# cielavenir/7bgzf

Hardware: NVIDIA B200
Metric: BGZF compress GB/s (uncompressed) (higher is better)
Workload: dtype u8

## Files before the change

7bgzf_b200/b200bgzf.py:

```python
import ctypes
import os

_HERE = os.path.dirname(os.path.abspath(__file__))
LIB_PATH = os.environ.get("B200BGZF_LIB_PATH") or os.path.join(_HERE, "lib7bgzf_b200.so")
HOOK_PATH = os.path.join(_HERE, "7bgzf.so")
APPLET_PATH = os.path.join(_HERE, "7bgzf")

BLOCK_SIZE = 0xFF00
MAX_BLOCK_SIZE = 0x10000
APPEND_EOF = 1
VERIFY = 2
FRAME_MIGZ = 4
E_NOFIT, E_ARG, E_CUDA, E_FORMAT, E_NOSPACE, E_CRC = 1, -1, -2, -3, -4, -5
EOF_BLOCK = bytes.fromhex("1f8b08040000000000ff0600424302001b0003000000000000000000")

EXPORTS = [
    "b200bgzf_create", "b200bgzf_destroy", "b200bgzf_strerror", "b200bgzf_last_error", "b200bgzf_compress_bound",
    "b200bgzf_compress_device", "b200bgzf_compress_host", "b200bgzf_compress_blocks_host", "b200bgzf_inflate_size_host",
    "b200bgzf_inflate_device", "b200bgzf_inflate_host", "b200bgzf_profile", "b200bgzf_launch_count", "b200bgzf_parse_method",
    "b200bgzf_host_alloc", "b200bgzf_host_free", "b200bgzf_member_header", "b200bgzf_compress_host_index", "b200bgzf_gzi_format",
    "b200bgzf_multi_create", "b200bgzf_multi_destroy", "b200bgzf_multi_count", "b200bgzf_multi_ctx", "b200bgzf_shard_blocks",
    "b200bgzf_multi_compress_bound", "b200bgzf_multi_compress_host", "b200bgzf_multi_inflate_host",
    "b200bgzf_pieces_gap_bytes", "b200bgzf_compress_pieces_host", "b200bgzf_crc32_combine", "b200bgzf_container_plan",
    "b200bgzf_container_head", "b200bgzf_container_bound", "b200bgzf_container_frame", "b200bgzf_container_compress_host",
# ... 107 lines not shown
    if rc != 0:
        raise B200BgzfError(rc, "container plan")
    return bs.value, sp


def container_frame(kind, param, stream, piece_off, piece_crc, in_bytes, lib=None):
    lib = lib or load()
    n = len(piece_off)
    head = lib.b200bgzf_container_head(kind, n)
    buf = bytearray(head + len(stream) + 64 + 40 * (n + 1))
    buf[head : head + len(stream)] = stream
    off = (ctypes.c_uint64 * max(n, 1))(*piece_off)
    crc = (ctypes.c_uint32 * max(n, 1))(*piece_crc)
    total = lib.b200bgzf_container_frame(kind, param, _addr(buf), len(buf), len(stream), off, crc, n, in_bytes)
    return bytes(buf[:total])


def _addr(buf):
    if isinstance(buf, int):
        return buf
    if isinstance(buf, bytes):
        return ctypes.cast(ctypes.c_char_p(buf), ctypes.c_void_p).value
    if hasattr(buf, "ctypes"):
        return buf.ctypes.data
    if hasattr(buf, "data_ptr"):
        return buf.data_ptr()
    return ctypes.addressof((ctypes.c_char * len(buf)).from_buffer(buf))


class Codec:

    def __init__(self, device=-1, path=LIB_PATH):
        self.lib = load(path)
        h = ctypes.c_void_p()
        rc = self.lib.b200bgzf_create(ctypes.byref(h), device)
        if rc != 0:
            raise B200BgzfError(rc, self.lib.b200bgzf_strerror(rc).decode())
        self.h = h

    def close(self):
        if self.h:
            self.lib.b200bgzf_destroy(self.h)
            self.h = None

    def __del__(self):
        try:
            self.close()
        except Exception:
            pass

    def _check(self, rc, ok=(0,)):
        if rc not in ok:
            raise B200BgzfError(rc, self.lib.b200bgzf_strerror(rc).decode() + " / " + self.lib.b200bgzf_last_error(self.h).decode())
        return rc

    def bound(self, n, block_size=BLOCK_SIZE):
        return self.lib.b200bgzf_compress_bound(n, block_size)

    def compress(self, data, level=6, block_size=BLOCK_SIZE, eof=True, flags=0):
        out = bytearray(self.bound(len(data), block_size))
        n = ctypes.c_size_t()
        self._check(self.lib.b200bgzf_compress_host(self.h, _addr(data) if len(data) else None, len(data), block_size, level,
                                                    _addr(out), len(out), ctypes.byref(n), (APPEND_EOF if eof else 0) | flags))
        return bytes(out[: n.value])

    def compress_pieces(self, data, spec, level=6, block_size=BLOCK_SIZE):
        nb = (len(data) + block_size - 1) // block_size
        cap = self.bound(len(data), block_size) + self.lib.b200bgzf_pieces_gap_bytes(len(data), block_size, ctypes.byref(spec))
        out = bytearray(cap)
        off = (ctypes.c_uint64 * max(nb, 1))()
        crc = (ctypes.c_uint32 * max(nb, 1))()
        n = ctypes.c_size_t()
        self._check(self.lib.b200bgzf_compress_pieces_host(self.h, _addr(data) if len(data) else None, len(data), block_size, level,
                                                           ctypes.byref(spec), _addr(out), len(out), ctypes.byref(n), off, crc, max(nb, 1)))
        return bytes(out[: n.value]), list(off[:nb]), list(crc[:nb])

    def container(self, kind, data, level=6, param=0):
        out = bytearray(self.lib.b200bgzf_container_bound(kind, param, len(data)))
        n = ctypes.c_size_t()
        self._check(self.lib.b200bgzf_container_compress_host(self.h, kind, param, _addr(data) if len(data) else None, len(data), level,
                                                              _addr(out), len(out), ctypes.byref(n)))
        return bytes(out[: n.value])

    def container_inflate(self, kind, blob, flags=0):
        total = ctypes.c_size_t()
        rc = self.lib.b200bgzf_container_inflate_size(kind, _addr(blob), len(blob), ctypes.byref(total), None)
        if rc != 0:
            raise B200BgzfError(rc, "container size")
        total = total.value
        out = bytearray(max(total, 1))
        n = ctypes.c_size_t()
        self._check(self.lib.b200bgzf_container_inflate_host(self.h, kind, _addr(blob), len(blob), _addr(out), len(out), ctypes.byref(n), flags))
        return bytes(out[: n.value])

    def inflate_units(self, blob, units, out_bytes, flags=0, want_crc=False):
        arr = (Unit * len(units))(*[Unit(*u) for u in units])
        out = bytearray(max(out_bytes, 1))
        n = ctypes.c_size_t()
        crc = (ctypes.c_uint32 * max(len(units), 1))() if want_crc else None
        self._check(self.lib.b200bgzf_inflate_units_host(self.h, _addr(blob), len(blob), arr, len(units), _addr(out), len(out), ctypes.byref(n), flags, crc))
        return (bytes(out[: n.value]), list(crc[: len(units)])) if want_crc else bytes(out[: n.value])

    def compress_indexed(self, data, level=6, block_size=BLOCK_SIZE, eof=True):
        nb = (len(data) + block_size - 1) // block_size
        out = bytearray(self.bound(len(data), block_size))
        off = (ctypes.c_uint64 * max(nb, 1))()
        n = ctypes.c_size_t()
        self._check(self.lib.b200bgzf_compress_host_index(self.h, _addr(data) if len(data) else None, len(data), block_size, level,
                                                          _addr(out), len(out), ctypes.byref(n), APPEND_EOF if eof else 0, off, nb))
        return bytes(out[: n.value]), list(off[:nb])

    def compress_into(self, src_addr, nbytes, dst_addr, dst_cap, level=6, block_size=BLOCK_SIZE, eof=True):
        n = ctypes.c_size_t()
        self._check(self.lib.b200bgzf_compress_host(self.h, src_addr, nbytes, block_size, level, dst_addr, dst_cap, ctypes.byref(n),
                                                    APPEND_EOF if eof else 0))
        return n.value

    def inflate(self, data, flags=0):
        total, nm = ctypes.c_size_t(), ctypes.c_size_t()
        self._check(self.lib.b200bgzf_inflate_size_host(_addr(data), len(data), ctypes.byref(total), ctypes.byref(nm)))
        out = bytearray(max(total.value, 1))
        n = ctypes.c_size_t()
        self._check(self.lib.b200bgzf_inflate_host(self.h, _addr(data), len(data), _addr(out), len(out), ctypes.byref(n), flags))
        return bytes(out[: n.value])

    def inflate_into(self, src_addr, nbytes, dst_addr, dst_cap, flags=0):
        n = ctypes.c_size_t()
        self._check(self.lib.b200bgzf_inflate_host(self.h, src_addr, nbytes, dst_addr, dst_cap, ctypes.byref(n), flags))
        return n.value

    def compress_blocks(self, payloads, level=6, caps=None):
        nb = len(payloads)
        srcs = (ctypes.c_void_p * nb)(*[_addr(p) if len(p) else None for p in payloads])
        slen = (ctypes.c_uint32 * nb)(*[len(p) for p in payloads])
        bufs = [bytearray(MAX_BLOCK_SIZE) for _ in range(nb)]
        dsts = (ctypes.c_void_p * nb)(*[_addr(b) for b in bufs])
        dlen = (ctypes.c_size_t * nb)(*(caps or [MAX_BLOCK_SIZE] * nb))
        st = (ctypes.c_int * nb)()
        rc = self.lib.b200bgzf_compress_blocks_host(self.h, srcs, slen, dsts, dlen, st, nb, level)
        self._check(rc, ok=(0, 1))
        return [bytes(bufs[i][: dlen[i]]) if st[i] == 0 else None for i in range(nb)], list(st)

    def compress_device(self, d_in, nbytes, d_out, out_cap, level=6, block_size=BLOCK_SIZE, eof=True, stream=None):
        n = ctypes.c_size_t()
        self._check(self.lib.b200bgzf_compress_device(self.h, d_in, nbytes, block_size, level, d_out, out_cap, ctypes.byref(n),
                                                      APPEND_EOF if eof else 0, stream))
        return n.value

    def inflate_device(self, d_in, nbytes, d_out, out_cap, flags=0, stream=None):
        n = ctypes.c_size_t()
        self._check(self.lib.b200bgzf_inflate_device(self.h, d_in, nbytes, d_out, out_cap, ctypes.byref(n), flags, stream))
        return n.value

    def profile(self, enable=True, reset=True):
        arr = (ctypes.c_ulonglong * 32)()
        self._check(self.lib.b200bgzf_profile(self.h, 1 if enable else 0, arr, 32, 1 if reset else 0))
        return list(arr)

    def launches(self):
        return self.lib.b200bgzf_launch_count(self.h)


class MultiCodec:

    def __init__(self, devices, path=LIB_PATH):
        self.lib = load(path)
        h = ctypes.c_void_p()
        arr = (ctypes.c_int * len(devices))(*devices)
        rc = self.lib.b200bgzf_multi_create(ctypes.byref(h), arr, len(devices))
        if rc != 0:
            raise B200BgzfError(rc, self.lib.b200bgzf_strerror(rc).decode())
        self.h = h

    def close(self):
        if self.h:
            self.lib.b200bgzf_multi_destroy(self.h)
            self.h = None

    def count(self):
        return self.lib.b200bgzf_multi_count(self.h)

    def bound(self, n, block_size=BLOCK_SIZE):
        return self.lib.b200bgzf_multi_compress_bound(self.h, n, block_size)

    def _check(self, rc):
        if rc != 0:
            raise B200BgzfError(rc, self.lib.b200bgzf_strerror(rc).decode())

    def compress_into(self, src_addr, nbytes, dst_addr, dst_cap, level=6, block_size=BLOCK_SIZE, eof=True, flags=0):
        n = ctypes.c_size_t()
        self._check(self.lib.b200bgzf_multi_compress_host(self.h, src_addr, nbytes, block_size, level, dst_addr, dst_cap, ctypes.byref(n),
                                                          (APPEND_EOF if eof else 0) | flags))
        return n.value

    def compress(self, data, level=6, block_size=BLOCK_SIZE, eof=True, flags=0):
        out = bytearray(self.bound(len(data), block_size))
        n = self.compress_into(_addr(data) if len(data) else None, len(data), _addr(out), len(out), level, block_size, eof, flags)
        return bytes(out[:n])

    def container(self, kind, data, level=6, param=0):
        out = bytearray(self.lib.b200bgzf_multi_container_bound(self.h, kind, param, len(data)))
        n = ctypes.c_size_t()
        self._check(self.lib.b200bgzf_multi_container_compress_host(self.h, kind, param, _addr(data) if len(data) else None, len(data), level,
                                                                    _addr(out), len(out), ctypes.byref(n)))
        return bytes(out[: n.value])

    def inflate_into(self, src_addr, nbytes, dst_addr, dst_cap, flags=0):
        n = ctypes.c_size_t()
        self._check(self.lib.b200bgzf_multi_inflate_host(self.h, src_addr, nbytes, dst_addr, dst_cap, ctypes.byref(n), flags))
        return n.value

    def inflate(self, data, flags=0):
        total, nm = ctypes.c_size_t(), ctypes.c_size_t()
        self._check(self.lib.b200bgzf_inflate_size_host(_addr(data), len(data), ctypes.byref(total), ctypes.byref(nm)))
        out = bytearray(max(total.value, 1))
        n = self.inflate_into(_addr(data), len(data), _addr(out), len(out), flags)
        return bytes(out[:n])


def shard_blocks(nblocks, shard, nshards, lib=None):
    lib = lib or load()
    a, b = ctypes.c_uint64(), ctypes.c_uint64()
    lib.b200bgzf_shard_blocks(nblocks, shard, nshards, ctypes.byref(a), ctypes.byref(b))
    return a.value, b.value


def member_header(data, lib=None):
    lib = lib or load()
    n = ctypes.c_uint64()
    h = lib.b200bgzf_member_header(_addr(data), len(data), ctypes.byref(n))
    return h, n.value


def gzi_format(caddr, uaddr, lib=None):
    lib = lib or load()
    n = len(caddr)
    ca, ua = (ctypes.c_uint64 * max(n, 1))(*caddr), (ctypes.c_uint64 * max(n, 1))(*uaddr)
    buf = bytearray(8 + 16 * max(n - 1, 0))
    w = lib.b200bgzf_gzi_format(ca, ua, n, _addr(buf), len(buf))
    return bytes(buf[:w])
```

7bgzf_b200/csrc/bgzf_compress.cu:

```cuda
#include <cuda_runtime.h>
#include <stdint.h>

#include <atomic>
#include <cstring>

#include "bgzf_block.h"
#include "bgzf_kernels.h"

#define SM_DATA 0u
#define SM_REGA (BG_DATA_BYTES)
#define SM_REGB (SM_REGA + 131072u)
#define SM_CRCTAB (SM_REGB + 32768u)
#define SM_LITFLAG (SM_CRCTAB + 1024u)
#define SM_SCAL (SM_LITFLAG + 256u)
#define SM_MBAR (SM_SCAL + 4u * BG_S_COUNT)
#define SM_FRONTIER (SM_MBAR + 8u)
#define SM_SCAN (SM_MBAR + 16u)
#define SM_READY (SM_SCAN + 4u * 36u)
#define SM_TOTAL (SM_READY + 128u)

extern "C" size_t bgzf_compress_smem_bytes(void) { return SM_TOTAL; }

__device__ __forceinline__ uint32_t smem_u32(const void *p) { return (uint32_t)__cvta_generic_to_shared(p); }

__device__ __forceinline__ void mbar_init(uint64_t *bar, uint32_t count)
{
    asm volatile("mbarrier.init.shared::cta.b64 [%0], %1;" ::"r"(smem_u32(bar)), "r"(count) : "memory");
}
__device__ __forceinline__ void mbar_expect_tx(uint64_t *bar, uint32_t bytes)
{
    asm volatile("mbarrier.arrive.expect_tx.shared::cta.b64 _, [%0], %1;" ::"r"(smem_u32(bar)), "r"(bytes) : "memory");
}
__device__ __forceinline__ void mbar_wait(uint64_t *bar, uint32_t parity)
{
    asm volatile(
        "{\n"
        ".reg .pred p;\n"
        "WAIT_%=:\n"
        "mbarrier.try_wait.parity.shared::cta.b64 p, [%0], %1;\n"
        "@p bra DONE_%=;\n"
        "bra WAIT_%=;\n"
        "DONE_%=:\n"
        "}\n" ::"r"(smem_u32(bar)), "r"(parity) : "memory");
}
__device__ __forceinline__ void tma_load_1d(void *dst_smem, const void *src_gmem, uint32_t bytes, uint64_t *bar)
{
    asm volatile("cp.async.bulk.shared::cluster.global.mbarrier::complete_tx::bytes [%0], [%1], %2, [%3];" ::"r"(smem_u32(dst_smem)),
                 "l"(src_gmem), "r"(bytes), "r"(smem_u32(bar))
                 : "memory");
}
__device__ __forceinline__ void fence_proxy_async()
{
    asm volatile("fence.proxy.async.shared::cta;" ::: "memory");
}

__device__ __forceinline__ unsigned hash_peers(uint32_t h, bool valid)
{
    unsigned peers = __ballot_sync(0xffffffffu, valid);
#pragma unroll
    for (int k = 0; k < BG_HASH_BITS; k++) {
        const uint32_t bit = (h >> k) & 1u;
        const unsigned b = __ballot_sync(0xffffffffu, bit != 0);
        peers &= b ^ (bit - 1u);
    }
    return peers;
}

__device__ __forceinline__ void build_peers_phase(const BgCtx &c, uint4 *notes, uint32_t lane, uint32_t warp, uint32_t nwarps, uint32_t first,
                                                  uint32_t step, uint4 *xprev, volatile uint8_t *ready)
{
    const uint32_t n = c.n, hb = c.scal[BG_S_HBYTES];
    const unsigned lt = (1u << lane) - 1u;
    const uint32_t ntiles = (n + 511u) >> 9;
    for (uint32_t tile = first + step * warp; tile < ntiles; tile += step * nwarps) {
        uint32_t w[4] = { 0xffffffffu, 0xffffffffu, 0xffffffffu, 0xffffffffu };
#pragma unroll
        for (uint32_t g = 0; g < 16; g++) {
            const uint32_t base = tile * 512u + g * 32u;
            if (base >= n) break;
            const uint32_t p = base + lane;
            const bool valid = p + hb <= n;
            const uint32_t h = valid ? bg_hash(c.dataw, p, hb) : BG_NOPOS;
            const unsigned peers = hash_peers(h, valid);
            uint32_t link = h;
            if (valid) {
                const unsigned lower = peers & lt;
                if (lower) {
                    link = base + (31u - (uint32_t)__clz(lower));
                } else {
                    const uint32_t note = 31u - (uint32_t)__clz(peers);
                    w[g >> 2] = (w[g >> 2] & ~(0xffu << (8 * (g & 3)))) | (note << (8 * (g & 3)));
                }
            }
            if (p < n) c.prev[p] = (uint16_t)link;
        }
        notes[tile * 32u + lane] = make_uint4(w[0], w[1], w[2], w[3]);
        if (xprev) {
            __syncwarp();
            const uint4 *ts = (const uint4 *)(c.prev + tile * 512u);
            xprev[tile * 64u + lane] = ts[lane];
            xprev[tile * 64u + 32u + lane] = ts[32u + lane];
        }
        if (ready) {
            __threadfence_block();
            __syncwarp();
            if (lane == 0) ready[tile] = 1;
        }
    }
}

__device__ __forceinline__ void import_peer_tiles(const BgCtx &c, const uint4 *xprev, uint32_t t, uint32_t rank, uint32_t parts)
{
    const uint32_t pieces = ((c.n + 511u) >> 9) * 64u;
    uint4 *dst = (uint4 *)c.prev;
    for (uint32_t i = t; i < pieces; i += BG_THREADS)
        if ((i >> 6) % parts != rank) dst[i] = __ldcg(xprev + i);
}

#define BG_LINKERS 4u
__device__ __forceinline__ void build_link_phase(const BgCtx &c, const uint4 *notes, uint32_t warp, uint32_t lane, volatile uint32_t *turn,
                                                 volatile uint8_t *ready)
{
    const uint32_t n = c.n;
    const uint32_t ntiles = (n + 511u) >> 9;
    volatile uint16_t *vhead = c.head;
    for (uint32_t tile = warp; tile < ntiles; tile += BG_LINKERS) {
        if (ready) {
            while (!ready[tile]) __nanosleep(40);
            __threadfence_block();
        }
        const uint4 cur = __ldcg(notes + tile * 32u + lane);
        const uint32_t w[4] = { cur.x, cur.y, cur.z, cur.w };
        uint32_t hs[16];
#pragma unroll
        for (uint32_t g = 0; g < 16; g++) {
            const uint32_t note = (w[g >> 2] >> (8 * (g & 3))) & 0xffu;
            hs[g] = note != 0xffu ? (uint32_t)c.prev[tile * 512u + g * 32u + lane] : 0xffffffffu;
        }
        while (*turn != tile) {}
        __threadfence_block();
        uint16_t old[16];
#pragma unroll
        for (uint32_t g = 0; g < 16; g++) {
            const uint32_t h = hs[g];
            if (h != 0xffffffffu) {
                const uint32_t note = (w[g >> 2] >> (8 * (g & 3))) & 31u;
                old[g] = vhead[h];
                vhead[h] = (uint16_t)(tile * 512u + g * 32u + note);
            }
        }
        __threadfence_block();
        __syncwarp();
        if (lane == 0) *turn = tile + 1;
#pragma unroll
        for (uint32_t g = 0; g < 16; g++)
            if (hs[g] != 0xffffffffu) c.prev[tile * 512u + g * 32u + lane] = old[g];
    }
}


__device__ __forceinline__ void mark_remote(uint32_t *local_word, uint32_t owner, uint32_t bits)
{
    uint32_t raddr;
    asm volatile("mapa.shared::cluster.u32 %0, %1, %2;" : "=r"(raddr) : "r"(smem_u32(local_word)), "r"(owner));
    asm volatile("red.relaxed.cluster.shared::cluster.or.b32 [%0], %1;" ::"r"(raddr), "r"(bits) : "memory");
}

template <bool SPLIT>
__device__ __forceinline__ void mark_bits(uint32_t *mark, uint32_t word, uint32_t bits, uint32_t own, uint32_t parts)
{
    BG_ASSERT(word < 2064u);
    if (!SPLIT) {
        atomicOr(&mark[word], bits);
        return;
    }
    const uint32_t owner = word % parts;
    if (owner == own) atomicOr(&mark[word], bits);
    else mark_remote(&mark[word], owner, bits);
    if (bits & 0xC0000000u) {
        const uint32_t next = (word + 1u) % parts;
        if (next == own) atomicOr(&mark[word], bits & 0xC0000000u);
        else if (next != owner) mark_remote(&mark[word], next, bits & 0xC0000000u);
    }
}

template <bool SPLIT, bool H3>
__device__ __forceinline__ void search_nearest_t(const BgCtx &c, uint32_t t, uint32_t own, uint32_t parts)
{
    const uint32_t n = c.n, lane = t & 31u;
    uint32_t *elig = (uint32_t *)(c.regb + BG_B_TODO), *mark = (uint32_t *)(c.regb + BG_B_MARK);
    const BgSearchPrm sp = bg_search_prm(c);
    if (sp.depth <= 1) {
        const uint32_t hist1 = bg_f_hist(c);
        for (uint32_t p = t; p < n; p += BG_THREADS) {
            if (SPLIT && (p >> 5) % parts != own) continue;
            bool deep;
            uint32_t target;
            c.R[p] = p < hist1 ? 0u : bg_nearest_t<H3>(c, sp, p, &deep, &target);
        }
        return;
    }
    const bool opt = c.prm.opt_passes > 0;
    const uint32_t hist = bg_f_hist(c);
    if (t == 0 && own == 0) mark_bits<SPLIT>(mark, hist >> 5, 1u << (hist & 31u), own, parts);
    for (uint32_t p0 = t - lane; p0 < n; p0 += BG_THREADS) {
        const uint32_t word = p0 >> 5;
        BG_ASSERT(word < 2048u);
        if (SPLIT && word % parts != own) continue;
        const uint32_t p = p0 + lane;
        if (p0 + 32u <= hist) {
            c.R[p] = 0;
            if (opt) ((uint4 *)c.cand)[p] = make_uint4(0u, 0u, 0u, 0u);
            continue;
        }
        bool deep = false;
        uint32_t target = p + 1, r = 0;
        const bool live = p < n && p >= hist;
        if (live) r = bg_nearest_t<H3>(c, sp, p, &deep, &target);
        if (p < n) c.R[p] = r;
        if (opt) {
            if (p < n) {
                const uint32_t k = r ? bg_off_bin(bg_mw_off(r)) : 4u;
                ((uint4 *)c.cand)[p] = make_uint4(k == 0 ? r : 0u, k == 1 ? r : 0u, k == 2 ? r : 0u, k == 3 ? r : 0u);
            }
            const unsigned em = __ballot_sync(0xffffffffu, deep);
            if (lane == 0) elig[word] = em;
            continue;
        }
        const bool lit = live && target == p + 1;
        const unsigned lm = __ballot_sync(0xffffffffu, lit), em = __ballot_sync(0xffffffffu, deep);
        const uint32_t before = __shfl_up_sync(0xffffffffu, target, 1);
        if (lane == 0) {
            elig[word] = em;
            if (lm << 1) mark_bits<SPLIT>(mark, word, lm << 1, own, parts);
            if (lm >> 31) mark_bits<SPLIT>(mark, word + 1, 1u, own, parts);
        }
        if (live && !lit && (lane == 0 || before != target)) mark_bits<SPLIT>(mark, target >> 5, 1u << (target & 31u), own, parts);
    }
}

template <bool SPLIT>
__device__ __forceinline__ void search_nearest(const BgCtx &c, uint32_t t, uint32_t own, uint32_t parts)
{
    if (c.scal[BG_S_HBYTES] == 3) search_nearest_t<SPLIT, true>(c, t, own, parts);
    else search_nearest_t<SPLIT, false>(c, t, own, parts);
}

template <bool H3>
__device__ __forceinline__ void drain_queue(const BgCtx &c, const uint32_t *queue, uint32_t from, uint32_t count, uint32_t lane)
{
    if (lane < count) {
        const uint32_t e = queue[from + lane];
        const uint32_t p = e >> 16, q = e & 0xffffu;
        BG_ASSERT(p < c.n && q < p && p - q <= 32768u);
        const uint32_t v = bg_deep_extend(c, H3, p, q);
        if (v) {
            atomicMax(&c.R[p], v);
            if (c.cand) atomicMax(&c.cand[4u * p + bg_off_bin(p - q)], v);
        }
    }
}

template <bool H3>
__device__ __forceinline__ void deep_batch(const BgCtx &c, uint32_t *queue, uint32_t &cnt, uint32_t p, bool active, uint32_t lane)
{
    uint32_t q = BG_NOPOS, b1 = 3, tail = 0;
    int depth = (int)c.scal[BG_S_DEPTH] - 1;
    const unsigned lt = (1u << lane) - 1u;
    uint32_t tmask = 0xffffffffu;
    if (active) {
        const uint32_t r1 = __ldcg(c.R + p);
        b1 = r1 ? r1 >> 16 : 3u;
        tmask = bg_tail_mask(H3, r1);
        tail = bg_ld32(c.dataw, p + b1 - 3u) & tmask;
        q = c.prev[c.prev[p]];
    }
    bool live = active && depth > 0 && bg_in_window(p, q);
    const uint32_t f4 = H3 && active ? bg_ld32(c.dataw, p) : 0u;
    int cap = 4 * depth;
    while (__any_sync(0xffffffffu, live)) {
#pragma unroll
        for (uint32_t k = 0; k < BG_SCAN_CHUNK_SHALLOW; k++) {
            bool pass = false;
            const uint32_t qc = q;
            if (live) {
                const uint32_t qn = c.prev[q];
                pass = (bg_ld32(c.dataw, q + b1 - 3u) & tmask) == tail;
                if (!H3 || bg_ld32(c.dataw, q) == f4) depth--;
                if (H3) cap--;
                q = qn;
                live = depth > 0 && (!H3 || cap > 0) && bg_in_window(p, q);
            }
            const unsigned m = __ballot_sync(0xffffffffu, pass);
            if (m) {
                BG_ASSERT(cnt + __popc(m) <= BG_QUEUE_WORDS_SHALLOW);
                if (pass) queue[cnt + __popc(m & lt)] = (p << 16) | qc;
                cnt += __popc(m);
            }
        }
        if (cnt >= 32u) {
            __syncwarp();
            do {
                cnt -= 32u;
                drain_queue<H3>(c, queue, cnt, 32u, lane);
            } while (cnt >= 32u);
            __syncwarp();
            if (live) {
                const uint32_t r = __ldcg(c.R + p);
                if ((r >> 16) > b1) {
// ... 242 lines not shown

__device__ __forceinline__ uint32_t chunk_class(const BgCtx &c, uint32_t ch)
{
    if (ch * BG_CHUNK >= c.n) return 0u;
    const uint32_t *sc = (const uint32_t *)(c.stepcode + ch * BG_CHUNK);
    uint32_t zeros = 0;
#pragma unroll
    for (uint32_t k = 0; k < BG_CHUNK / 4u; k++) {
        const uint32_t v = sc[k];
        zeros += __popc((v - 0x01010101u) & ~v & 0x80808080u);
    }
    return zeros >= 64u ? 7u : zeros >> 3;
}

__device__ __forceinline__ void chunk_order_count(const BgCtx &c, uint32_t t, uint32_t &cls, uint32_t &rank)
{
    const uint32_t lane = t & 31u, warp = t >> 5;
    uint32_t *cnt = (uint32_t *)(c.regb + BG_B_CLASSCNT);
    cls = chunk_class(c, t);
    rank = 0;
#pragma unroll
    for (uint32_t k = 0; k < 8u; k++) {
        const unsigned m = __ballot_sync(0xffffffffu, cls == k);
        if (cls == k) rank = __popc(m & ((1u << lane) - 1u));
        if (lane == k) cnt[k * 32u + warp] = __popc(m);
    }
}

__device__ __forceinline__ void chunk_order_scan(const BgCtx &c, uint32_t t)
{
    if (t >= 32u) return;
    uint32_t *cnt = (uint32_t *)(c.regb + BG_B_CLASSCNT);
    uint32_t v[8], sum = 0;
#pragma unroll
    for (uint32_t k = 0; k < 8u; k++) { v[k] = cnt[t * 8u + k]; sum += v[k]; }
    uint32_t inc = sum;
    for (int d = 1; d < 32; d <<= 1) {
        const uint32_t y = __shfl_up_sync(0xffffffffu, inc, d);
        if (t >= (uint32_t)d) inc += y;
    }
    uint32_t run = inc - sum;
#pragma unroll
    for (uint32_t k = 0; k < 8u; k++) { cnt[t * 8u + k] = run; run += v[k]; }
}

__device__ __forceinline__ void chunk_order_place(const BgCtx &c, uint32_t t, uint32_t cls, uint32_t rank)
{
    const uint32_t *cnt = (const uint32_t *)(c.regb + BG_B_CLASSCNT);
    BG_ASSERT(cls < 8u && cnt[cls * 32u + (t >> 5)] + rank < BG_MAX_CHUNKS);
    ((uint16_t *)(c.regb + BG_B_PERM))[cnt[cls * 32u + (t >> 5)] + rank] = (uint16_t)t;
}

__device__ __forceinline__ void bitonic_sort_512(uint32_t *keys, uint32_t t)
{
    for (uint32_t k = 2; k <= 512; k <<= 1) {
        for (uint32_t j = k >> 1; j > 0; j >>= 1) {
            if (t < 512) {
                uint32_t x = t ^ j;
                if (x > t) {
                    uint32_t a = keys[t], b = keys[x];
                    bool up = (t & k) == 0;
                    if ((a > b) == up) { keys[t] = b; keys[x] = a; }
                }
            }
            __syncthreads();
        }
    }
}

__device__ __forceinline__ uint32_t block_exclusive_scan_1024(uint32_t *v, uint32_t *scratch, uint32_t t)
{
    const uint32_t lane = t & 31u, warp = t >> 5;
    uint32_t x = v[t], inc = x;
    for (int d = 1; d < 32; d <<= 1) {
        uint32_t y = __shfl_up_sync(0xffffffffu, inc, d);
        if (lane >= (uint32_t)d) inc += y;
    }
    if (lane == 31) scratch[warp] = inc;
    __syncthreads();
    if (warp == 0) {
        uint32_t w = scratch[lane], winc = w;
        for (int d = 1; d < 32; d <<= 1) {
            uint32_t y = __shfl_up_sync(0xffffffffu, winc, d);
            if (lane >= (uint32_t)d) winc += y;
        }
        scratch[lane] = winc - w;
        if (lane == 31) scratch[32] = winc;
    }
    __syncthreads();
    v[t] = scratch[warp] + inc - x;
    uint32_t total = scratch[32];
    __syncthreads();
    return total;
}

__device__ __forceinline__ void gather_member(const uint32_t *src, uint32_t n, uint8_t *dst, uint32_t t, uint32_t nthr)
{
    const uint32_t head = (uint32_t)((4u - ((uintptr_t)dst & 3u)) & 3u);
    if (n <= head + 4) {
        for (uint32_t i = t; i < n; i += nthr) dst[i] = (uint8_t)(__ldcg(src + (i >> 2)) >> (8u * (i & 3u)));
        return;
    }
    if (t < head) dst[t] = (uint8_t)(__ldcg(src) >> (8u * t));
    const uint32_t words = (n - head) >> 2;
    uint32_t *dw = (uint32_t *)(dst + head);
    const uint32_t sh = head * 8u;
    for (uint32_t i = t; i < words; i += nthr)
        dw[i] = __funnelshift_r(__ldcg(src + i), __ldcg(src + i + 1), sh);
    const uint32_t done = head + words * 4u;
    if (t < n - done) dst[done + t] = (uint8_t)(__ldcg(src + ((done + t) >> 2)) >> (8u * ((done + t) & 3u)));
}

__device__ __forceinline__ uint32_t block_exclusive_scan_1024(uint32_t *v, uint32_t *scratch, uint32_t t);

__device__ __forceinline__ void fused_compaction(const BgzfCompressArgs &a, uint32_t *v, uint32_t *scratch, uint32_t t)
{
    uint64_t carry = *a.gather_total;
    for (uint32_t start = 0; start < a.nblocks; start += 1024u) {
        const uint32_t i = start + t;
        v[t] = i < a.nblocks ? __ldcg(a.out_len + i) : 0u;
        __syncthreads();
        const uint32_t total = block_exclusive_scan_1024(v, scratch, t);
        if (i < a.nblocks) a.gather_off[i] = carry + v[t];
        carry += total;
        __syncthreads();
    }
    if (t == 0) *a.gather_total = carry;
    __syncthreads();
    const uint32_t grp = t >> 8, gt = t & 255u;
    for (uint32_t b = grp; b < a.nblocks; b += BG_THREADS / 256u) {
        BG_ASSERT(__ldcg(a.out_len + b) <= BG_SLOT_BYTES && a.gather_off[b] + __ldcg(a.out_len + b) <= carry);
        gather_member((const uint32_t *)(a.slots + (size_t)b * BG_SLOT_BYTES), __ldcg(a.out_len + b), a.gather_out + a.gather_off[b], gt, 256u);
    }
}

#define PROF_MARK(i)                                                        \
    do {                                                                    \
        if (prof && t == 0) {                                               \
            long long now_ = clock64();                                     \
            atomicAdd((unsigned long long *)&prof[i], (unsigned long long)(now_ - tprev_)); \
            tprev_ = now_;                                                  \
        }                                                                   \
    } while (0)

template <bool SPLIT>
__device__ __forceinline__ void compress_blocks(BgzfCompressArgs &a)
{
    extern __shared__ __align__(128) uint8_t smem[];
    const uint32_t t = threadIdx.x, T = BG_THREADS;
    uint64_t *mbar = (uint64_t *)(smem + SM_MBAR);
    uint32_t *scan_scratch = (uint32_t *)(smem + SM_SCAN);
    unsigned long long *prof = a.prof;
    long long tprev_ = prof ? clock64() : 0;

    BgCtx c;
    c.dataw = (uint32_t *)(smem + SM_DATA);
    c.prev = (uint16_t *)(smem + SM_REGA);
    c.stepcode = smem + SM_REGA;
    c.jump8 = smem + SM_REGA + 65536u;
    c.offarr = (uint16_t *)(smem + SM_REGA + 65536u);
    c.head = (uint16_t *)(smem + SM_REGB);
    c.regb = smem + SM_REGB;
    c.crctab = (uint32_t *)(smem + SM_CRCTAB);
    c.litflag = smem + SM_LITFLAG;
    c.scal = (uint32_t *)(smem + SM_SCAL);
    const uint32_t crank = SPLIT ? cluster_rank() : 0u, csize = SPLIT ? cluster_size() : 1u;
    const uint32_t unit = SPLIT ? blockIdx.x / csize : blockIdx.x;
    uint32_t *const unit_scratch = a.scratch + (size_t)unit * (SPLIT ? BGZF_SCRATCH_WORDS + BGZF_SPLIT_EXTRA_WORDS : BGZF_SCRATCH_WORDS);
    c.R = unit_scratch;
    c.cand = a.cand ? a.cand + (size_t)unit * (4u * BG_MAX_BLOCK) : nullptr;
    c.crcpow = a.crcpow;
    c.prm = a.prm;
    c.frame = bg_frame(a.hdr_bytes ? a.hdr_bytes : 18u, 8u, 1u, 0u);
    c.perm = (const uint16_t *)(smem + SM_REGB + BG_B_PERM);

    if (t < 256) c.crctab[t] = a.crctab[t];
    if (t == 0) {
        mbar_init(mbar, 1);
        asm volatile("fence.mbarrier_init.release.cluster;" ::: "memory");
    }
    __syncthreads();
    uint32_t parity = 0;

    for (uint32_t b = unit; b < a.nblocks; b += SPLIT ? a.nblocks : gridDim.x) {
        const uint8_t *src;
        uint32_t n;
        if (a.in_off) {
            src = a.in + a.in_off[b];
            n = a.in_len[b];
        } else {
            const uint64_t off = (uint64_t)b * a.block_size;
            src = a.in + off;
            const uint64_t rem = a.in_bytes - off;
            n = rem < a.block_size ? (uint32_t)rem : a.block_size;
        }
        c.out = (uint32_t *)(a.slots + (size_t)b * BG_SLOT_BYTES);
        if (a.piece_mode) {
            const uint64_t gb = a.piece_base + b;
            const bool first = gb % a.member_blocks == 0, last = (gb + 1) % a.member_blocks == 0 || gb + 1 == a.piece_total;
            uint32_t hist = 0;
            if (a.history && !first && !a.in_off) {
                const uint64_t in_member = (gb % a.member_blocks) * a.block_size, in_buffer = (uint64_t)a.lead + (uint64_t)b * a.block_size;
                uint64_t h = in_member < in_buffer ? in_member : in_buffer;
                if (h > a.history) h = a.history;
                hist = (uint32_t)h - (uint32_t)h % BG_HISTORY_STEP;
            }
            src -= hist;
            n += hist;
            c.frame = bg_frame(first ? a.head_gap : 0u, last ? a.tail_gap : 0u, last && !a.no_final ? 1u : 0u, 1u, hist);
        }
        c.n = n;

        const bool aligned = (((uintptr_t)src) & 15u) == 0;
        const uint32_t bulk = aligned ? (n & ~15u) : 0u;
        if (bulk) {
            if (t == 0) {
                fence_proxy_async();
                mbar_expect_tx(mbar, bulk);
                tma_load_1d(smem + SM_DATA, src, bulk, mbar);
            }
        }
        for (uint32_t i = bulk + t; i < n; i += T)
            smem[SM_DATA + i] = src[i];
        bg_phase_init(c, t, T);
        if (bulk) {
            mbar_wait(mbar, parity);
            parity ^= 1u;
        }
        __syncthreads();
        PROF_MARK(0);

        bg_phase_scan(c, t, T);
        __syncthreads();
        bg_phase_count(c, t, T);
        __syncthreads();
        bg_phase_settle(c, t, T);
        __syncthreads();
        PROF_MARK(1);
        PROF_MARK(2);
        uint4 *hi = (uint4 *)(c.R + BG_MAX_BLOCK + 32);
        if (SPLIT) {
            uint4 *xprev = (uint4 *)(unit_scratch + BGZF_SCRATCH_WORDS);
            build_peers_phase(c, hi, t & 31u, t >> 5, BG_THREADS / 32u, crank, csize, xprev, nullptr);
            cluster_sync();
            import_peer_tiles(c, xprev, t, crank, csize);
            __syncthreads();
            PROF_MARK(3);
            if (t < 32u * BG_LINKERS) build_link_phase(c, hi, t >> 5, t & 31u, &c.scal[BG_S_WLIST], nullptr);
        } else {
            volatile uint8_t *ready = (volatile uint8_t *)(smem + SM_READY);
            if (t < 128u) ready[t] = 0;
            __syncthreads();
            if (t < 32u * BG_LINKERS) build_link_phase(c, hi, t >> 5, t & 31u, &c.scal[BG_S_WLIST], ready);
            else build_peers_phase(c, hi, t & 31u, (t >> 5) - BG_LINKERS, BG_THREADS / 32u - BG_LINKERS, 0u, 1u, nullptr, ready);
        }
        __syncthreads();
        PROF_MARK(10);
        {
            bg_phase_search_clear(c, t, T);
            if (SPLIT) cluster_sync();
            else __syncthreads();
            search_nearest<SPLIT>(c, t, crank, csize);
            if (SPLIT) cluster_sync();
            else __syncthreads();
            PROF_MARK(21);
            if (c.scal[BG_S_DEPTH] > 1) {
                bg_phase_search_todo(c, t, T, crank, csize);
                __syncthreads();
                const bool h3 = c.scal[BG_S_HBYTES] == 3;
                if (c.scal[BG_S_DEPTH] <= 24u) {
                    if (h3) search_deep_batches<true>(c, t, crank, csize);
                    else search_deep_batches<false>(c, t, crank, csize);
                } else {
                    if (h3) search_deep<true>(c, t, crank, csize);
                    else search_deep<false>(c, t, crank, csize);
                }
            }
        }
        if (SPLIT) {
            cluster_sync();
            if (crank) return;
        }
        __syncthreads();
        PROF_MARK(4);
        for (int pass = 0; pass <= c.prm.opt_passes; pass++) {
            if (pass == 0) {
                bg_phase_accept(c, t, T);
            } else {
                bg_phase_costs(c, t, T);
                __syncthreads();
                dp_segment_warp(c, t >> 5, t & 31u, (uint32_t *)(smem + SM_REGA + 65536u) + (t >> 5) * BG_DP_RING);
            }
            __syncthreads();
            if (bg_f_hist(c)) {
                bg_phase_history_steps(c, t, T);
                __syncthreads();
            }
            PROF_MARK(15);
            bg_phase_jump(c, t, T);
            __syncthreads();
            PROF_MARK(5);
            bg_phase_walk_clear(c, t, T);
            bg_phase_clear_freq(c, t, T);
            __syncthreads();
            bg_phase_walk_mark(c, t, T);
            __syncthreads();
            bg_phase_walk_list(c, t, T);
            __syncthreads();
            PROF_MARK(16);
            bg_phase_walk_a(c, t, T);
            __syncthreads();
            PROF_MARK(17);
            bg_phase_walk_b(c, t, T);
            uint32_t ccls, crnk;
            chunk_order_count(c, t, ccls, crnk);
            __syncthreads();
            PROF_MARK(18);
            bg_phase_walk_c(c, t, T);
            chunk_order_scan(c, t);
            __syncthreads();
            chunk_order_place(c, t, ccls, crnk);
            __syncthreads();
            PROF_MARK(6);
            bg_phase_tally(c, t, T);
            __syncthreads();
            bg_phase_lkeys(c, t, T);
            __syncthreads();
            PROF_MARK(7);
            bitonic_sort_512((uint32_t *)(c.regb + BG_B_KEYS), t);
            PROF_MARK(11);
            bg_phase_huff_prep(c, t, T);
            __syncthreads();
            bg_phase_huff(c, t, T);
            __syncthreads();
            bg_phase_huff_depth(c, t, T);
            __syncthreads();
            bg_phase_huff_fix(c, t, T);
            __syncthreads();
            bg_phase_huff_assign(c, t, T);
            __syncthreads();
            PROF_MARK(12);
        }
        bg_phase_hdr1(c, t, T);
        __syncthreads();
        bg_phase_hdr2(c, t, T);
        __syncthreads();
        bg_phase_hdr3(c, t, T);
        __syncthreads();
        const uint32_t nitems = block_exclusive_scan_1024((uint32_t *)(c.regb + BG_B_CBITS), scan_scratch, t);
        bg_phase_hdr4(c, t, T);
        __syncthreads();
        bg_phase_hdr4b(c, t, T);
        __syncthreads();
        bg_phase_hdr5(c, t, T, nitems);
        __syncthreads();
        PROF_MARK(13);
        bg_phase_decide_b(c, t, T);
        __syncthreads();
        bg_phase_codes_a(c, t, T);
        __syncthreads();
        bg_phase_codes_b(c, t, T);
        __syncthreads();
        bg_phase_codes_c(c, t, T);
        __syncthreads();
        bg_phase_tabs(c, t, T);
        __syncthreads();
        PROF_MARK(8);
        bg_phase_hdr_bits(c, t, T);
        bg_phase_sizes(c, t, T);
        __syncthreads();
        PROF_MARK(19);
        block_exclusive_scan_1024((uint32_t *)(c.regb + BG_B_CBITS), scan_scratch, t);
        block_exclusive_scan_1024((uint32_t *)(c.regb + BG_B_IOFF), scan_scratch, t);
        PROF_MARK(20);
        bg_phase_zero_out(c, t, T);
        __syncthreads();
        PROF_MARK(14);
        bg_phase_emit(c, t, T);
        if (t == 0) {
            const uint32_t st = c.scal[BG_S_STATUS];
            a.out_len[b] = st ? 0u : bg_f_hdr(c) + c.scal[BG_S_PAYLOAD] + bg_f_trl(c);
            if (a.crc_out) a.crc_out[b] = c.scal[BG_S_CRC];
            a.status[b] = st;
            if (st) atomicOr(a.err_flag, 1u);
        }
        fence_proxy_async();
        __syncthreads();
        PROF_MARK(9);
    }
    if (!SPLIT && a.gather_out) {
        __threadfence();
        __syncthreads();
        if (t == 0) scan_scratch[35] = atomicAdd(a.done_count, 1u) == gridDim.x - 1u ? 1u : 0u;
        __syncthreads();
        if (scan_scratch[35]) {
            __threadfence();
            fused_compaction(a, (uint32_t *)(smem + SM_REGB), scan_scratch, t);
        }
    }
}

__global__ void __launch_bounds__(BG_THREADS, 1)
bgzf_compress_kernel(BgzfCompressArgs a)
{
    compress_blocks<false>(a);
}

__global__ void __launch_bounds__(BG_THREADS, 1)
bgzf_compress_split_kernel(BgzfCompressArgs a)
{
    compress_blocks<true>(a);
}

__global__ void __launch_bounds__(1024, 1)
bgzf_scan_kernel(const uint32_t *len, uint64_t *off, uint32_t nmax, const uint64_t *count_dev, const uint64_t *base_dev,
                 uint64_t *total_out)
{
// ... 125 lines not shown
```

7bgzf_b200/csrc/bgzf_kernels.h:

```cpp
#ifndef BGZF_KERNELS_H
#define BGZF_KERNELS_H
#include <cuda_runtime.h>
#include <stdint.h>

#include "bgzf_block.h"

#define BGZF_SCRATCH_WORDS (65536u + 32u + 16384u + 32u)
#define BGZF_SPLIT_EXTRA_WORDS 32768u
#define BGZF_SPLIT_MAX 8
#define BGZF_PROF_SLOTS 32

struct BgzfCompressArgs {
    const uint8_t *in;
    const uint64_t *in_off;
    const uint32_t *in_len;
    uint64_t in_bytes;
    uint32_t block_size;
    uint32_t nblocks;
    uint32_t hdr_bytes;
    BgParams prm;
    uint8_t *slots;
    uint32_t *out_len;
    uint32_t *status;
    uint32_t *err_flag;
    uint32_t *scratch;
    uint32_t *cand;
    const uint32_t *crctab;
    const uint32_t *crcpow;
    unsigned long long *prof;
    uint8_t *gather_out;
    uint64_t *gather_off;
    uint64_t *gather_total;
    uint32_t *done_count;
    uint32_t piece_mode;
    uint32_t member_blocks;
    uint64_t piece_base;
    uint64_t piece_total;
    uint32_t head_gap;
    uint32_t tail_gap;
    uint32_t no_final;
    uint32_t *crc_out;
    uint32_t history;
    uint32_t lead;
};

struct BgzfInflateArgs {
    const uint8_t *in;
    const uint64_t *in_off;
    const uint64_t *out_off;
    const uint32_t *hdr_len;
    const uint32_t *msize;
    const uint32_t *unit_isize;
    uint32_t *unit_crc;
    uint32_t nblocks;
    uint8_t *out;
    uint32_t *status;
    uint32_t *err_flag;
    int verify_crc;
    const uint32_t *crctab;
    const uint32_t *crcpow;
};

struct BgzfIndexWork {
    uint32_t max_blocks;
    uint32_t *tile_count;
    uint64_t *tile_off;
    uint64_t *cand_off;
    uint32_t *jump, *jump2;
    uint32_t *reach;
    uint64_t *pick_idx;
    uint64_t *in_off;
    uint64_t *out_off;
    uint32_t *isize;
    uint64_t *ncand, *nmembers, *out_bytes;
    uint32_t *status;
};

#ifdef __cplusplus
extern "C" {
#endif
size_t bgzf_compress_smem_bytes(void);
cudaError_t bgzf_launch_compress(const BgzfCompressArgs *a, int grid, cudaStream_t stream);
cudaError_t bgzf_launch_compress_split(const BgzfCompressArgs *a, int csize, cudaStream_t stream);
cudaError_t bgzf_launch_scan(const uint32_t *len, uint64_t *off, uint32_t nmax, const uint64_t *count_dev,
                             const uint64_t *base_dev, uint64_t *total_out, cudaStream_t stream);
cudaError_t bgzf_launch_compact(const uint8_t *slots, const uint32_t *len, uint64_t *off, uint32_t nblocks, uint8_t *out,
                                uint64_t *total, int append_eof, cudaStream_t stream);
cudaError_t bgzf_launch_deliver(const uint8_t *slots, const uint32_t *len, const uint64_t *out_off, uint8_t *host_out, uint32_t n,
                                cudaStream_t stream);
size_t bgzf_index_tiles(uint64_t in_bytes);
#define BGZF_INDEX_LAUNCHES 8
cudaError_t bgzf_launch_index(const uint8_t *in, uint64_t in_bytes, const BgzfIndexWork *w, cudaStream_t stream);
cudaError_t bgzf_launch_inflate(const BgzfInflateArgs *a, cudaStream_t stream);
#ifdef __cplusplus
}
#endif
#endif
```

Before: 29.37.

## Streamline hash-chain linking with branchless sink writes and acquire/release turn handoff

The hash-peer ballot loop becomes inline PTX that fuses the bit test, vote and mask update. A branchless masked hash covers all supported widths. The serialized linker phase packs hash and position into one op word and sends invalid entries to a dummy sink slot in shared memory, so every lane stores unconditionally. Acquire/release shared-memory ops replace the volatile spin plus thread fences on the turn counter. Optional per-tile profiling counters are also added, which widens the profile buffer and puts extra branches in the hot path.

```diff
diff --git a/7bgzf_b200/b200bgzf.py b/7bgzf_b200/b200bgzf.py
--- a/7bgzf_b200/b200bgzf.py
+++ b/7bgzf_b200/b200bgzf.py
@@ -283,9 +283,9 @@
         self._check(self.lib.b200bgzf_inflate_device(self.h, d_in, nbytes, d_out, out_cap, ctypes.byref(n), flags, stream))
         return n.value
 
-    def profile(self, enable=True, reset=True):
-        arr = (ctypes.c_ulonglong * 32)()
-        self._check(self.lib.b200bgzf_profile(self.h, 1 if enable else 0, arr, 32, 1 if reset else 0))
+    def profile(self, enable=True, reset=True, slots=32):
+        arr = (ctypes.c_ulonglong * slots)()
+        self._check(self.lib.b200bgzf_profile(self.h, 1 if enable else 0, arr, slots, 1 if reset else 0))
         return list(arr)
 
     def launches(self):
diff --git a/7bgzf_b200/csrc/bgzf_compress.cu b/7bgzf_b200/csrc/bgzf_compress.cu
--- a/7bgzf_b200/csrc/bgzf_compress.cu
+++ b/7bgzf_b200/csrc/bgzf_compress.cu
@@ -59,17 +59,30 @@
     unsigned peers = __ballot_sync(0xffffffffu, valid);
 #pragma unroll
     for (int k = 0; k < BG_HASH_BITS; k++) {
-        const uint32_t bit = (h >> k) & 1u;
-        const unsigned b = __ballot_sync(0xffffffffu, bit != 0);
-        peers &= b ^ (bit - 1u);
+        asm volatile("{\n\t.reg .pred p;\n\t.reg .b32 b, t;\n\t"
+                     "and.b32 t, %1, %2;\n\t"
+                     "setp.ne.u32 p, t, 0;\n\t"
+                     "vote.sync.ballot.b32 b, p, 0xffffffff;\n\t"
+                     "selp.b32 t, -1, 0, p;\n\t"
+                     "lop3.b32 %0, %0, b, t, 0x90;\n\t}"
+                     : "+r"(peers)
+                     : "r"(h), "r"(1u << k));
     }
     return peers;
 }
 
+__device__ __forceinline__ uint32_t hash_any_width(const uint32_t *dataw, uint32_t p, uint32_t m0, uint32_t m1)
+{
+    const uint32_t v0 = bg_ld32(dataw, p) & m0, v1 = bg_ld32(dataw, p + 4u) & m1;
+    return ((v0 * 0x1E35A7BDu) ^ (v1 * 0x9E3779B1u)) >> (32 - BG_HASH_BITS);
+}
+
 __device__ __forceinline__ void build_peers_phase(const BgCtx &c, uint4 *notes, uint32_t lane, uint32_t warp, uint32_t nwarps, uint32_t first,
-                                                  uint32_t step, uint4 *xprev, volatile uint8_t *ready)
+                                                  uint32_t step, uint4 *xprev, volatile uint8_t *ready, unsigned long long *prof, long long t0)
 {
     const uint32_t n = c.n, hb = c.scal[BG_S_HBYTES];
+    const uint32_t m0 = hb == 3 ? 0xffffffu : 0xffffffffu, m1 = hb == 8 ? 0xffffffffu : hb == 5 ? 0xffu : 0u;
+    BG_ASSERT(hb == 3 || hb == 4 || hb == 5 || hb == 8);
     const unsigned lt = (1u << lane) - 1u;
     const uint32_t ntiles = (n + 511u) >> 9;
     for (uint32_t tile = first + step * warp; tile < ntiles; tile += step * nwarps) {
@@ -80,7 +93,7 @@
             if (base >= n) break;
             const uint32_t p = base + lane;
             const bool valid = p + hb <= n;
-            const uint32_t h = valid ? bg_hash(c.dataw, p, hb) : BG_NOPOS;
+            const uint32_t h = valid ? hash_any_width(c.dataw, p, m0, m1) : BG_NOPOS;
             const unsigned peers = hash_peers(h, valid);
             uint32_t link = h;
             if (valid) {
@@ -105,6 +118,7 @@
             __threadfence_block();
             __syncwarp();
             if (lane == 0) ready[tile] = 1;
+            if (prof && lane == 0) atomicAdd(&prof[BGZF_PROF_READY + tile], (unsigned long long)(clock64() - t0));
         }
     }
 }
@@ -118,43 +132,63 @@
 }
 
 #define BG_LINKERS 4u
+#define BG_LINK_SINK (SM_SCAN + 4u * 33u - SM_REGB)
+__device__ __forceinline__ uint32_t ld_acquire_cta(const volatile uint32_t *p)
+{
+    uint32_t v;
+    asm volatile("ld.acquire.cta.shared::cta.u32 %0, [%1];" : "=r"(v) : "r"(smem_u32((const void *)p)) : "memory");
+    return v;
+}
+__device__ __forceinline__ void st_release_cta(volatile uint32_t *p, uint32_t v)
+{
+    asm volatile("st.release.cta.shared::cta.u32 [%0], %1;" ::"r"(smem_u32((const void *)p)), "r"(v) : "memory");
+}
 __device__ __forceinline__ void build_link_phase(const BgCtx &c, const uint4 *notes, uint32_t warp, uint32_t lane, volatile uint32_t *turn,
-                                                 volatile uint8_t *ready)
+                                                 volatile uint8_t *ready, unsigned long long *prof, long long t0)
 {
     const uint32_t n = c.n;
     const uint32_t ntiles = (n + 511u) >> 9;
-    volatile uint16_t *vhead = c.head;
+    volatile uint8_t *vhead = (volatile uint8_t *)c.head;
+    static_assert(BG_LINK_SINK >= 2u * BG_HASH_SIZE && BG_LINK_SINK < 65536u, "the sink lies outside head[] and within 16 bits");
     for (uint32_t tile = warp; tile < ntiles; tile += BG_LINKERS) {
+        BG_ASSERT(tile < 128u);
+        const long long w0 = prof ? clock64() : 0;
         if (ready) {
             while (!ready[tile]) __nanosleep(40);
             __threadfence_block();
         }
+        const long long w1 = prof ? clock64() : 0;
         const uint4 cur = __ldcg(notes + tile * 32u + lane);
         const uint32_t w[4] = { cur.x, cur.y, cur.z, cur.w };
-        uint32_t hs[16];
+        uint32_t op[16];
 #pragma unroll
         for (uint32_t g = 0; g < 16; g++) {
             const uint32_t note = (w[g >> 2] >> (8 * (g & 3))) & 0xffu;
-            hs[g] = note != 0xffu ? (uint32_t)c.prev[tile * 512u + g * 32u + lane] : 0xffffffffu;
-        }
-        while (*turn != tile) {}
-        __threadfence_block();
-        uint16_t old[16];
+            const uint32_t h = c.prev[tile * 512u + g * 32u + lane];
+            BG_ASSERT(note == 0xffu || h < BG_HASH_SIZE);
+            op[g] = note != 0xffu ? (h << 17) | (tile * 512u + g * 32u + note) : BG_LINK_SINK << 16;
+        }
+        const long long w2 = prof ? clock64() : 0;
+        while (ld_acquire_cta(turn) != tile) {}
+        const long long w3 = prof ? clock64() : 0;
+        uint32_t old[16];
 #pragma unroll
         for (uint32_t g = 0; g < 16; g++) {
-            const uint32_t h = hs[g];
-            if (h != 0xffffffffu) {
-                const uint32_t note = (w[g >> 2] >> (8 * (g & 3))) & 31u;
-                old[g] = vhead[h];
-                vhead[h] = (uint16_t)(tile * 512u + g * 32u + note);
-            }
-        }
-        __threadfence_block();
+            volatile uint16_t *slot = (volatile uint16_t *)(vhead + (op[g] >> 16));
+            old[g] = *slot;
+            *slot = (uint16_t)op[g];
+        }
         __syncwarp();
-        if (lane == 0) *turn = tile + 1;
+        if (lane == 0) st_release_cta(turn, tile + 1);
+        if (prof && lane == 0) {
+            atomicAdd(&prof[23], (unsigned long long)(w1 - w0));
+            atomicAdd(&prof[24], (unsigned long long)(w3 - w2));
+            atomicAdd(&prof[BGZF_PROF_TURN + tile], (unsigned long long)(w3 - t0));
+            if (tile + 1 == ntiles) atomicAdd(&prof[25], (unsigned long long)(clock64() - t0));
+        }
 #pragma unroll
         for (uint32_t g = 0; g < 16; g++)
-            if (hs[g] != 0xffffffffu) c.prev[tile * 512u + g * 32u + lane] = old[g];
+            if ((op[g] >> 16) != BG_LINK_SINK) c.prev[tile * 512u + g * 32u + lane] = (uint16_t)old[g];
     }
 }
 
@@ -703,6 +737,7 @@
     uint32_t *scan_scratch = (uint32_t *)(smem + SM_SCAN);
     unsigned long long *prof = a.prof;
     long long tprev_ = prof ? clock64() : 0;
+    uint32_t *const pscr = scan_scratch;
 
     BgCtx c;
     c.dataw = (uint32_t *)(smem + SM_DATA);
@@ -792,18 +827,24 @@
         uint4 *hi = (uint4 *)(c.R + BG_MAX_BLOCK + 32);
         if (SPLIT) {
             uint4 *xprev = (uint4 *)(unit_scratch + BGZF_SCRATCH_WORDS);
-            build_peers_phase(c, hi, t & 31u, t >> 5, BG_THREADS / 32u, crank, csize, xprev, nullptr);
+            build_peers_phase(c, hi, t & 31u, t >> 5, BG_THREADS / 32u, crank, csize, xprev, nullptr, nullptr, 0);
             cluster_sync();
             import_peer_tiles(c, xprev, t, crank, csize);
             __syncthreads();
             PROF_MARK(3);
-            if (t < 32u * BG_LINKERS) build_link_phase(c, hi, t >> 5, t & 31u, &c.scal[BG_S_WLIST], nullptr);
+            if (t < 32u * BG_LINKERS) build_link_phase(c, hi, t >> 5, t & 31u, &c.scal[BG_S_WLIST], nullptr, nullptr, 0);
         } else {
             volatile uint8_t *ready = (volatile uint8_t *)(smem + SM_READY);
             if (t < 128u) ready[t] = 0;
-            __syncthreads();
-            if (t < 32u * BG_LINKERS) build_link_phase(c, hi, t >> 5, t & 31u, &c.scal[BG_S_WLIST], ready);
-            else build_peers_phase(c, hi, t & 31u, (t >> 5) - BG_LINKERS, BG_THREADS / 32u - BG_LINKERS, 0u, 1u, nullptr, ready);
+            if (prof && t == 0) { pscr[0] = 0; pscr[1] = 0; pscr[2] = 0xffffffffu; }
+            __syncthreads();
+            const long long t0 = prof ? clock64() : 0;
+            if (t < 32u * BG_LINKERS) {
+                build_link_phase(c, hi, t >> 5, t & 31u, &c.scal[BG_S_WLIST], ready, prof, t0);
+            } else {
+                build_peers_phase(c, hi, t & 31u, (t >> 5) - BG_LINKERS, BG_THREADS / 32u - BG_LINKERS, 0u, 1u, nullptr, ready, prof, t0);
+                if (prof && (t & 31u) == 0) atomicMax(&pscr[0], (uint32_t)(clock64() - t0));
+            }
         }
         __syncthreads();
         PROF_MARK(10);
@@ -811,9 +852,20 @@
             bg_phase_search_clear(c, t, T);
             if (SPLIT) cluster_sync();
             else __syncthreads();
+            const long long t1 = prof ? clock64() : 0;
             search_nearest<SPLIT>(c, t, crank, csize);
+            if (!SPLIT && prof && (t & 31u) == 0) {
+                const uint32_t d = (uint32_t)(clock64() - t1);
+                atomicMax(&pscr[1], d);
+                atomicMin(&pscr[2], d);
+            }
             if (SPLIT) cluster_sync();
             else __syncthreads();
+            if (!SPLIT && prof && t == 0) {
+                atomicAdd(&prof[22], (unsigned long long)pscr[0]);
+                atomicAdd(&prof[26], (unsigned long long)pscr[1]);
+                atomicAdd(&prof[27], (unsigned long long)pscr[2]);
+            }
             PROF_MARK(21);
             if (c.scal[BG_S_DEPTH] > 1) {
                 bg_phase_search_todo(c, t, T, crank, csize);
diff --git a/7bgzf_b200/csrc/bgzf_kernels.h b/7bgzf_b200/csrc/bgzf_kernels.h
--- a/7bgzf_b200/csrc/bgzf_kernels.h
+++ b/7bgzf_b200/csrc/bgzf_kernels.h
@@ -8,7 +8,9 @@
 #define BGZF_SCRATCH_WORDS (65536u + 32u + 16384u + 32u)
 #define BGZF_SPLIT_EXTRA_WORDS 32768u
 #define BGZF_SPLIT_MAX 8
-#define BGZF_PROF_SLOTS 32
+#define BGZF_PROF_SLOTS 288
+#define BGZF_PROF_TURN 32
+#define BGZF_PROF_READY 160
 
 struct BgzfCompressArgs {
     const uint8_t *in;
```

Measured after the change: 33.15, median of 6. 12.9% higher.
